# edwardyang12/Dex-NERF

Hardware: AMD Instinct MI355X
Metric: rays/sec (64+128 samples) + PSNR vs ref, 400x400 scene (higher is better)
Workload: dtype bf16; 1 GPU; C2 render: 400x400 rays/step/GPU, 64 coarse + 128 fine samples, coarse+fine FlexibleNeRFModel D8/W256/skip4 + viewdirs, PE L=10/4, 20 Dex thresholds, validation mode (det. resampling, no noise)

## Files before the change

### dex-nerf_amd/csrc/mlp_device.h

```cpp
#pragma once
#include <cstdlib>
#include <utility>

#include "mlp_layout.h"

namespace dn {

typedef float f32x16 __attribute__((ext_vector_type(16)));
typedef float f32x4 __attribute__((ext_vector_type(4)));
typedef __bf16 bf16x8 __attribute__((ext_vector_type(8)));
typedef _Float16 f16x8 __attribute__((ext_vector_type(8)));

template <int N, class F, int... I>
__device__ __forceinline__ void static_for_impl(F&& f, std::integer_sequence<int, I...>) {
  (f(std::integral_constant<int, I>{}), ...);
}
template <int N, class F>
__device__ __forceinline__ void static_for(F&& f) {
  static_for_impl<N>(static_cast<F&&>(f), std::make_integer_sequence<int, N>{});
}

constexpr int kRingPhases = 5;
constexpr int kSlotBytes = kPhasePieces * kPieceBytes;
constexpr int kRingBytes = kRingPhases * kSlotBytes;
constexpr int kInRows = 10;

template <int BF16> struct Prec;
template <> struct Prec<1> {
  using BPiece = bf16x8;
  using Elem = __bf16;
  static constexpr int EPP = 8;
  static constexpr int PPT = 2;
};
template <> struct Prec<2> {
  using BPiece = f16x8;
  using Elem = _Float16;
  static constexpr int EPP = 8;
  static constexpr int PPT = 2;
};
template <> struct Prec<0> {
  using BPiece = f32x4;
  using Elem = float;
  static constexpr int EPP = 4;
  static constexpr int PPT = 4;
};
template <int BF16, int PT> constexpr int waves_of() { return (BF16 && PT == 1) ? 8 : 4; }

struct FwdParams {
  const char* packed;
  int bias_bytes;
  int total_pieces;
  int D;
  unsigned skip_mask;
  int use_viewdirs;
  int mode;
  const float* rays;
  int ray_stride;
  const float* z;
// ... 131 lines not shown
      rd_cur = rd_nxt;
      rd_nxt = ring + slot_nxt * kSlotBytes + lane16;
    }
  }

  __device__ __forceinline__ void mid_phase() {
    if constexpr (WAVES == 8 && G::LEADER_DMA) dma_phase(pend_src + PER_WAVE * kPieceBytes, pend_dst + PER_WAVE * kPieceBytes, wave < 4 ? 1u : 0u);
    else if constexpr (WAVES == 8) dma_phase(pend_src, pend_dst, wave >= 4 ? 1u : 0u);
  }

  template <bool EVEN>
  __device__ __forceinline__ void phase_begin2() {
    if constexpr (EVEN) {
      asm volatile("s_waitcnt vmcnt(0)" ::: "memory");
      __builtin_amdgcn_s_barrier();
      advance_issue();
      dma_phase(pend_src, pend_dst, wave < 4 ? 1u : 0u);
      dma_phase(pend_src + PER_WAVE * kPieceBytes, pend_dst + PER_WAVE * kPieceBytes, wave < 4 ? 1u : 0u);
    }
    slot_nxt = (slot_nxt + 1 == kRingPhases) ? 0 : slot_nxt + 1;
    rda_cur = slot_cur_base + lane16;
    slot_cur_base = __builtin_amdgcn_readfirstlane(ring_addr + slot_nxt * kSlotBytes);
  }
  template <bool EVEN>
  __device__ __forceinline__ void mid_phase2() {
    if constexpr (EVEN) {
      advance_issue();
      dma_phase(pend_src, pend_dst, wave < 4 ? 1u : 0u);
      dma_phase(pend_src + PER_WAVE * kPieceBytes, pend_dst + PER_WAVE * kPieceBytes, wave < 4 ? 1u : 0u);
    }
  }
  unsigned long long xs_src[2];
  unsigned xs_dst[2];
  template <int PERIOD>
  __device__ __forceinline__ void xs_period_begin() {
    static_assert(PERIOD == kPhasePieces || PERIOD == 2 * kPhasePieces, "barrier period: one or two phases");
    if constexpr (PERIOD == 2 * kPhasePieces) asm volatile("s_waitcnt vmcnt(0)" ::: "memory");
    else asm volatile("s_waitcnt vmcnt(8)" ::: "memory");
    __builtin_amdgcn_s_barrier();
#pragma unroll
    for (int h = 0; h < PERIOD / kPhasePieces; ++h) {
      advance_issue();
      const unsigned long long bits = reinterpret_cast<unsigned long long>(wsrc + pend_src);
      const unsigned lo = __builtin_amdgcn_readfirstlane(static_cast<unsigned>(bits));
      const unsigned hi = __builtin_amdgcn_readfirstlane(static_cast<unsigned>(bits >> 32));
      xs_src[h] = (static_cast<unsigned long long>(hi) << 32) | lo;
      xs_dst[h] = __builtin_amdgcn_readfirstlane(ring_addr + pend_dst);
    }
  }
  template <int PERIOD, int Q>
  __device__ __forceinline__ void xs_dma_step() {
    constexpr int STEPS = PERIOD / 8;
    constexpr int H = (Q % STEPS) / 2;
    constexpr int OFF = (Q % 2) * 2048;
    unsigned keep;
    asm volatile(
        "s_cmp_lg_u32 %[wave], %[who]\n\t"
        "s_cbranch_scc1 .Ldn_xs_skip%=\n\t"
        "s_mov_b32 %[keep], m0\n\t"
        "s_mov_b32 m0, %[lds]\n\t"
        "s_nop 1\n\t"
        "global_load_lds_dwordx4 %[voff], %[sbase] offset:%[o0]\n\t"
        "global_load_lds_dwordx4 %[voff], %[sbase] offset:%[o1]\n\t"
        "s_mov_b32 m0, %[keep]\n"
        ".Ldn_xs_skip%=:"
        : [keep] "=&s"(keep)
        : [wave] "s"(wave), [who] "n"(Q / STEPS), [lds] "s"(xs_dst[H]), [voff] "v"(lane16), [sbase] "s"(xs_src[H]), [o0] "n"(OFF), [o1] "n"(OFF + 1024)
        : "memory", "scc");
  }
  template <int PERIOD, int POS>
  __device__ __forceinline__ void at_position_xs() {
    if constexpr (POS % PERIOD == 0) xs_period_begin<PERIOD>();
    if constexpr (POS % kPhasePieces == 0) {
      slot_nxt = (slot_nxt + 1 == kRingPhases) ? 0 : slot_nxt + 1;
      rda_cur = slot_cur_base + lane16;
      slot_cur_base = __builtin_amdgcn_readfirstlane(ring_addr + slot_nxt * kSlotBytes);
    }
  }
  template <int PERIOD, int POS>
  __device__ __forceinline__ void xs_after_piece() {
    if constexpr ((POS % PERIOD) < PERIOD / 2) xs_dma_step<PERIOD, POS % PERIOD>();
  }
  template <int PH, int POS>
  __device__ __forceinline__ void at_position() {
    static_assert(PH == kPhasePieces || (G::ASM_READS && G::LEADER_DMA), "the two-phase barrier period is the 48-point geometry's");
    if constexpr (POS % kPhasePieces == 0) {
      if constexpr (PH == 2 * kPhasePieces) phase_begin2<(POS % PH) == 0>();
      else phase_begin();
    }
    if constexpr (POS % kPhasePieces == kPhasePieces / 2) {
      if constexpr (PH == 2 * kPhasePieces) mid_phase2<(POS % PH) == kPhasePieces / 2>();
      else mid_phase();
    }
  }

  template <int POS, int N, int PH = kPhasePieces, bool BIAS = true>
  __device__ __forceinline__ void skip() {
    static_for<N>([&](auto i_c) {
      constexpr int pos = POS + decltype(i_c)::value;
      static_assert(pos % kPhasePieces != 0 || decltype(i_c)::value == 0, "padding never crosses a phase");
      if constexpr (pos % kPhasePieces == kPhasePieces / 2) at_position<PH, pos>();
      if constexpr (!G::ASM_READS || decltype(i_c)::value >= N - G::PREFETCH) prefetch<pos>();
    });
    settle<BIAS>();
  }

  template <int PERIOD, int POS, int N>
  __device__ __forceinline__ void skip_xs() {
    static_for<N>([&](auto i_c) {
      constexpr int pos = POS + decltype(i_c)::value;
      static_assert(pos % kPhasePieces != 0 || decltype(i_c)::value == 0, "padding never crosses a phase");
      static_assert(pos % PERIOD != 0, "padding never opens a barrier period");
      xs_after_piece<PERIOD, pos>();
      if constexpr (decltype(i_c)::value >= N - G::PREFETCH) prefetch<pos>();
    });
    settle<true>();
  }

  template <int POS>
  __device__ __forceinline__ void prefetch() {
    constexpr int q = (POS % kPhasePieces) + G::PREFETCH;
    if constexpr (G::ASM_READS) {
      const unsigned base = (q < kPhasePieces) ? rda_cur : slot_cur_base + lane16;
      asm volatile("ds_read_b128 %0, %1 offset:%2" : "=v"(af[POS % G::PREFETCH]) : "v"(base), "n"((q % kPhasePieces) * kPieceBytes));
    } else {
      const char* base = (q < kPhasePieces) ? rd_cur : rd_nxt;
      af[POS % G::PREFETCH] = *reinterpret_cast<const f32x4*>(base + (q % kPhasePieces) * kPieceBytes);
    }
  }

  template <int E>
  __device__ __forceinline__ void prologue_read() {
    asm volatile("ds_read_b128 %0, %1 offset:%2" : "=v"(af[E]) : "v"(slot_cur_base + lane16), "n"(E * kPieceBytes));
  }
  template <int POS, int NEWER>
  __device__ __forceinline__ f32x4 take() {
    asm volatile("s_waitcnt lgkmcnt(%1)" : "+v"(af[POS % G::PREFETCH]) : "n"(NEWER));
    return af[POS % G::PREFETCH];
  }
  template <int OFF>
  __device__ __forceinline__ void bias_prefetch(unsigned addr) {
    asm volatile("ds_read_b128 %0, %1 offset:%2" : "=v"(bias_nxt) : "v"(addr), "n"(OFF));
  }
  template <int NEWER>
  __device__ __forceinline__ f32x4 bias_take() {
    asm volatile("s_waitcnt lgkmcnt(%1)" : "+v"(bias_nxt) : "n"(NEWER));
// ... 266 lines not shown
```

### dex-nerf_amd/csrc/mlp_fused48_kernel.h

```cpp
#pragma once
#include "mlp_stage48.h"

namespace dn {


template <bool MAY_BE_IDENTITY = true>
__device__ __forceinline__ float pe_value(float xc, f32x4 entry) {
  const float rev = __builtin_amdgcn_fractf(xc * entry[0]) + entry[1];
  const float s = __builtin_amdgcn_sinf(rev);
  if constexpr (MAY_BE_IDENTITY) return entry[2] * xc + entry[3] * s;
  else return s;
}

__device__ __forceinline__ void rotate3(const float (&x)[3], int g, float (&xr)[3]) {
  const unsigned r = static_cast<unsigned>(g) % 3u;
  const unsigned m1 = 0u - (r & 1u), m2 = 0u - (r >> 1);
  const unsigned b0 = __float_as_uint(x[0]), b1 = __float_as_uint(x[1]), b2 = __float_as_uint(x[2]);
  xr[0] = __uint_as_float(b0 ^ ((b0 ^ b1) & m1) ^ ((b0 ^ b2) & m2));
  xr[1] = __uint_as_float(b1 ^ ((b1 ^ b2) & m1) ^ ((b1 ^ b0) & m2));
  xr[2] = __uint_as_float(b2 ^ ((b2 ^ b0) & m1) ^ ((b2 ^ b1) & m2));
}

template <int W, int F, int DC = 0, unsigned MASKC = 0, int VIEWC = 0, int SAVE = 0, int OVLP = 0, int COMP = 0>
__global__ __launch_bounds__(kG48Waves * 64, 2) void mlp_forward48_kernel(FwdParams p, G48Params q) {
// ... 76 lines not shown
    const int ln = fresh_lane();
    int pt = tile * PPG + wave * PPW + ln;
    pt = pt < n_points ? pt : n_points - 1;
    const float* r = p.rays + static_cast<long long>(pt / p.S) * p.ray_stride;
#pragma unroll
    for (int c = 0; c < 6; ++c) dma4_lanes48(r + c, inbuf_addr + c * (PPW * 4));
    dma4_lanes48(p.z + pt, inbuf_addr + 6 * (PPW * 4));
#pragma unroll
    for (int c = 0; c < 3; ++c) dma4_lanes48(r + 8 + c, inbuf_addr + (7 + c) * (PPW * 4) + set * (3 * PPW * 4));
  };

  Pipe48<WAVES> pipe;
  pipe.ring = ring;
  pipe.ring_addr = static_cast<unsigned>(reinterpret_cast<uintptr_t>((__attribute__((address_space(3))) char*)ring));
  pipe.lane16 = lane * 16;
  pipe.wsrc = q.base + q.bias_bytes + kG48TableBytes;
  pipe.total_bytes = static_cast<unsigned>(q.total_pieces) * kPieceBytes;
  pipe.q_issue = 0;
  pipe.slot_wr = 0;
  pipe.wave = wave;
#pragma unroll
  for (int ph = 0; ph < (PH == kPhasePieces ? kRingPhases - 1 : kRingPhases - 2); ++ph) pipe.issue_phase();
  if constexpr (PH == kPhasePieces) {
    g48_prologue_wait(wave);
    __builtin_amdgcn_s_barrier();
  } else {
    asm volatile("s_waitcnt vmcnt(0) lgkmcnt(0)" ::: "memory");
    __syncthreads();
  }
  pipe.slot_nxt = 0;
  auto bias_at = [&](int tile) { return pipe.ring_addr + kRingBytes + ((fresh_lane() >> 4) << 4) + tile * 64; };
  pipe.rda_cur = pipe.ring_addr + lane * 16;
  pipe.slot_cur_base = pipe.ring_addr;
  static_for<PipeGeo48::PREFETCH - 1>([&](auto e_c) { pipe.template prologue_read<decltype(e_c)::value>(); });
  pipe.template bias_prefetch<0>(bias_at(0));
  pipe.template prologue_read<PipeGeo48::PREFETCH - 1>();

  unsigned trk = 0;
  int vset = 0;
  float tfreq[OVL ? 16 : 1], tphase[OVL ? 16 : 1], tw_id[3], tw_sin[3];
  float xr_n[PT][3];
  BP8 encp;
  if constexpr (OVL) {
    const f32x4* tabx = reinterpret_cast<const f32x4*>(tab_lds) + (lane >> 4) * 16;
#pragma unroll
    for (int u = 0; u < 16; ++u) {
      const f32x4 e = tabx[u];
      tfreq[u] = e[0]; tphase[u] = e[1];
      if (u < 3) { tw_id[u] = e[2]; tw_sin[u] = e[3]; }
    }
  }
  unsigned long long idm[3] = {0ull, 0ull, 0ull};
  if constexpr (OVX) {
    const f32x4* tabx = reinterpret_cast<const f32x4*>(tab_lds) + (lane >> 4) * 16;
#pragma unroll
    for (int u = 0; u < 3; ++u) idm[u] = __ballot(tabx[u][2] != 0.0f);
  }
  const int n_tiles = static_cast<int>(p.n_tiles);
  for (int tile = blockIdx.x; tile < n_tiles; tile += gridDim.x, vset = (VSETS == 2 ? vset ^ 1 : (vset == 2 ? 0 : vset + 1))) {
    const char* act_grp[PT] = {};
    const char* mask_base = nullptr;
    if constexpr (SAVE != 0) {
      const long long wt = static_cast<long long>(tile) * WAVES + wave;
#pragma unroll
      for (int t = 0; t < PT; ++t) {
        const long long G = wt * PT + t;
        act_grp[t] = uniform_ptr(p.act + ((G >> 1) * p.act_pieces * 2 + (G & 1)) * kPieceBytes);
      }
      mask_base = uniform_ptr(p.masks + wt * p.mask_words * (2 * kPieceBytes));
    }
    const bool first_tile = tile == static_cast<int>(blockIdx.x);
    if ((!OVL && !OVX) || first_tile) {
      const int ln = fresh_lane();
      const int j = ln & 15;
      const f32x4* tabx = reinterpret_cast<const f32x4*>(tab_lds) + (ln >> 4) * 16;
      char* pex = pex_of(ln);
      if (wave >= 4) asm volatile("s_waitcnt vmcnt(0)" ::: "memory");
      float in[PT][7];
#pragma unroll
      for (int t = 0; t < PT; ++t)
#pragma unroll
        for (int c = 0; c < 7; ++c) in[t][c] = inbuf[c * PPW + t * 16 + j];
      asm volatile("s_waitcnt lgkmcnt(0)" ::: "memory");
      {
        const int nxt = tile + gridDim.x;
        if (nxt < n_tiles) issue_inputs(nxt, vset ^ 1);
      }
#pragma unroll
      for (int t = 0; t < PT; ++t) {
        float x[3];
#pragma unroll
// ... 54 lines not shown
          maskw[t][nt >> 3] = mw;
        }
      }
    };
    auto unit_tail = [&](auto nt_c, auto t_c, const auto& bo, int slot0) {
      if constexpr (SAVE != 0) {
        constexpr int nt = decltype(nt_c)::value;
        if constexpr (nt % 4 == 3) save_unit(t_c, slot0 + nt / 4, bo[nt / 2 - 1], bo[nt / 2]);
      }
    };
    auto mask_store = [&](int stage) {
      if constexpr (SAVE != 0) {
        store16_uniform_at(mask_base, static_cast<unsigned>(stage) * (2 * kPieceBytes), pipe.lane16, make_uint4(maskw[0][0], maskw[0][1], maskw[1][0], maskw[1][1]));
        if constexpr (PT == 3)
          store16_uniform_at(mask_base, static_cast<unsigned>(stage) * (2 * kPieceBytes) + kPieceBytes, pipe.lane16, make_uint4(maskw[PT - 1][0], maskw[PT - 1][1], 0u, 0u));
      }
    };
    constexpr int KHU = KH / 2;

    BP8 ba[PT][KH], bb[PT][KH];
    int bias_tile = 0;
    float out4[PT][4];
    if constexpr (XS) {
      static_assert(DC >= 2 && KDP == 1, "a trunk behind layer1; the view-direction panel is one piece");
      constexpr int PX = PH;
      f32x4 pacc[PT];
      auto nothing = [&](auto) {};
      {
        BP8 pe[PT][KXP];
#pragma unroll
        for (int t = 0; t < PT; ++t)
#pragma unroll
          for (int k = 0; k < KXP; ++k) pe[t][k] = pe_xyz(t, k);
        run_stage48x<F, PX, NT, KXP, 0, 0, false, 0, 6, 0, 0>(pipe, pe, no_pe, bias_at(0), 0u, pacc,
            [&](auto nt_c, auto s_c) { hidden_op48<F, false, decltype(nt_c)::value, decltype(s_c)::value>(pacc, ba); }, nothing);
      }
      bias_tile += NT;
      static_for<DC - 1>([&](auto i_c) {
        constexpr int i = decltype(i_c)::value;
        constexpr int P0 = xs_trunk_pos(i, NT, KH, KXP, MASKC) % PX;
        auto& bin = (i % 2 == 0) ? ba : bb;
        auto& bout = (i % 2 == 0) ? bb : ba;
        auto ops = [&](auto nt_c, auto s_c) { hidden_op48<F, true, decltype(nt_c)::value, decltype(s_c)::value>(pacc, bout); };
        auto pend = [&](auto s_c) { hidden_op48<F, (i > 0), NT - 1, decltype(s_c)::value>(pacc, bin); };
        constexpr int PN = i > 0 ? 12 : 6;
        constexpr int BY = (NT - 1) / 2;
        if constexpr ((MASKC >> i) & 1u) {
          BP8 pe[PT][KXP];
#pragma unroll
          for (int t = 0; t < PT; ++t)
#pragma unroll
            for (int k = 0; k < KXP; ++k) pe[t][k] = pe_xyz(t, k);
          run_stage48x<F, PX, NT, KH, KXP, P0, false, 0, 12, PN, BY, (i == 0 ? 2 : 1)>(pipe, bin, [&](int t, int k) { return pe[t][k]; }, bias_at(bias_tile), 0u, pacc, ops, pend, &trk);
        } else {
          run_stage48x<F, PX, NT, KH, 0, P0, false, 0, 12, PN, BY, (i == 0 ? 2 : 1)>(pipe, bin, no_pe, bias_at(bias_tile), 0u, pacc, ops, pend, &trk);
        }
        bias_tile += NT;
      });
      auto& hx = ((DC - 1) % 2 == 0) ? ba : bb;
      auto& hy = ((DC - 1) % 2 == 0) ? bb : ba;
      constexpr int POS_A = xs_trunk_pos(DC - 1, NT, KH, KXP, MASKC) % PX;
      run_stage48x<F, PX, 1, KH, 0, POS_A, false, 0, 3, (DC > 1 ? 12 : 6), (NT - 1) / 2>(pipe, hx, no_pe, bias_at(bias_tile), 0u, pacc,
          [&](auto, auto s_c) { constexpr int t = decltype(s_c)::value; pick_op48(out4[t][3], pacc[t][0]); },
          [&](auto s_c) { hidden_op48<F, (DC > 1), NT - 1, decltype(s_c)::value>(pacc, hx); });
      constexpr int POS_F = (POS_A + KH) % PX;
      run_stage48x<F, PX, NT, KH, 0, POS_F, false, 0, 12, 3, KH, 1>(pipe, hx, no_pe, bias_at(bias_tile + 1), 0u, pacc,
          [&](auto nt_c, auto s_c) { hidden_op48<F, true, decltype(nt_c)::value, decltype(s_c)::value>(pacc, hy); },
          [&](auto s_c) { constexpr int t = decltype(s_c)::value; pick_op48(out4[t][3], pacc[t][0]); }, &trk);
      bias_tile += NT + 1;
      __builtin_amdgcn_sched_barrier(0);
      {
        const int ln = fresh_lane();
        const int j = ln & 15;
        const f32x4* tabd = reinterpret_cast<const f32x4*>(tab_lds + 1024) + (ln >> 4) * 8;
        char* pex = pex_of(ln);
        static_for<PT>([&](auto t_c) {
          constexpr int t = decltype(t_c)::value;
          float v[3];
#pragma unroll
          for (int c = 0; c < 3; ++c) v[c] = inbuf[(7 + 3 * vset + c) * PPW + t * 16 + j];
          float vr[3];
          rotate3(v, ln >> 4, vr);
          BP8 piece;
#pragma unroll
          for (int e = 0; e < 8; ++e) piece[e] = static_cast<Elem>((e < 3) ? pe_value<true>(vr[e % 3], tabd[e]) : pe_value<false>(vr[e % 3], tabd[e]));
          *reinterpret_cast<BP8*>(pex + t * kPieceBytes) = piece;
          __builtin_amdgcn_sched_barrier(0);
        });
      }
      __builtin_amdgcn_sched_barrier(0);
      constexpr int POS_D = (POS_F + NT * KH) % PX;
      constexpr int KT_D = KH + KDP;
      BP8 bg[PT][KH / 2];
      BP8 ped[PT];
      typedef float f32x2 __attribute__((ext_vector_type(2)));
      float ev[2] = {0.0f, 0.0f};
      f32x2 tbl[2] = {{0.0f, 0.0f}, {0.0f, 0.0f}};
      unsigned tab_addr_v = 0u, stash_addr_v = 0u;
      float in_n[PT][7];
      if constexpr (OVX) {
        static_assert(kEncOps <= enc_begin((NT / 2) * KT_D, KT_D), "the view-direction stage has a gap for every encoding op");
        {
          const unsigned must_wait = __builtin_amdgcn_readfirstlane(wave >= 4 ? 1u : 0u);
          asm volatile("s_cmp_eq_u32 %0, 0\n\t"
                       "s_cbranch_scc1 .Ldn_ovx_nowait%=\n\t"
                       "s_waitcnt vmcnt(0)\n"
                       ".Ldn_ovx_nowait%=:" ::"s"(must_wait) : "scc", "memory");
        }
        const int ln = fresh_lane();
        const int j = ln & 15;
#pragma unroll
        for (int t = 0; t < PT; ++t)
#pragma unroll
          for (int c = 0; c < 7; ++c) in_n[t][c] = inbuf[c * PPW + t * 16 + j];
        tab_addr_v = pipe.ring_addr + kRingBytes + static_cast<unsigned>(q.bias_bytes) + static_cast<unsigned>(ln >> 4) * 256u;
        stash_addr_v = pipe.ring_addr + kRingBytes + static_cast<unsigned>(q.bias_bytes) + kG48TableBytes + wave * (PT * KXP * kPieceBytes) + static_cast<unsigned>(ln) * 16u;
        asm volatile("ds_read_b64 %0, %1" : "=v"(tbl[0]) : "v"(tab_addr_v));
      }
#pragma unroll
      for (int t = 0; t < PT; ++t) ped[t] = *reinterpret_cast<const BP8*>(pex_of(pipe.lane16 >> 4) + t * kPieceBytes);
      asm volatile("s_waitcnt lgkmcnt(0)" : "+v"(ped[0]), "+v"(ped[1]), "+v"(ped[2]), "+v"(pipe.af[0]), "+v"(pipe.af[1]), "+v"(pipe.bias_nxt), "+v"(tbl[0]));
      if constexpr (OVX) {
        const int t2 = tile + 2 * static_cast<int>(gridDim.x);
        issue_inputs_flat(t2 < n_tiles ? t2 : tile, vset);
        const int ln = fresh_lane();
#pragma unroll
        for (int t = 0; t < PT; ++t) {
          float x[3];
#pragma unroll
          for (int c = 0; c < 3; ++c) x[c] = in_n[t][c] + in_n[t][3 + c] * in_n[t][6];
          rotate3(x, ln >> 4, xr_n[t]);
        }
      }
      auto enc_hook = [&](auto b_c, auto w_c) {
        if constexpr (OVX) {
          constexpr int b = decltype(b_c)::value, w = decltype(w_c)::value;
          constexpr int q0 = enc_begin(b, KT_D), cap = enc_cap(b, KT_D);
          auto one = [&](auto q_c) {
            constexpr int qq = decltype(q_c)::value;
            if constexpr (qq < kEncOps) {
              constexpr int mt = enc_table_slot_at(qq);
// ... 3 lines not shown
              if constexpr (mt >= 0) {
                f32x2& dst = tbl[mt & 1];
                asm volatile("ds_read_b64 %0, %1 offset:%2" : "=v"(dst) : "v"(ta), "n"((mt % 16) * 16));
              }
              const float xc = xr_n[tq][u % 3];
              float& val = ev[e & 1];
              const f32x2 entry = tbl[m & 1];
              if constexpr (kind == kEncMul) asm volatile("v_mul_f32 %0, %1, %2" : "=v"(val) : "v"(xc), "v"(entry[0]));
              else if constexpr (kind == kEncFract) asm volatile("v_fract_f32 %0, %0" : "+v"(val));
              else if constexpr (kind == kEncAdd) asm volatile("v_add_f32 %0, %0, %1" : "+v"(val) : "v"(entry[1]));
              else if constexpr (kind == kEncSin) asm volatile("v_sin_f32 %0, %0" : "+v"(val));
              else if constexpr (kind == kEncSel) {
                const unsigned long long im = idm[u < 3 ? u : 0];
                asm volatile("v_cndmask_b32 %0, %0, %1, %2" : "+v"(val) : "v"(xc), "s"(im));
              } else if constexpr (kind == kEncCvt) {
                typedef unsigned u32x4 __attribute__((ext_vector_type(4)));
                const float lo = ev[0], hi = ev[1];
                unsigned dw;
                if constexpr (F == 1) asm volatile("v_cvt_pk_bf16_f32 %0, %1, %2" : "=v"(dw) : "v"(lo), "v"(hi));
                else asm volatile("v_cvt_pk_f16_f32 %0, %1, %2" : "=v"(dw) : "v"(lo), "v"(hi));
                u32x4 pw = __builtin_bit_cast(u32x4, encp);
                pw[e / 2] = dw;
                encp = __builtin_bit_cast(BP8, pw);
              } else {
                const BP8 piece = encp;
                asm volatile("ds_write_b128 %0, %1 offset:%2" : : "v"(sa), "v"(piece), "n"((tq * KXP + k2) * kPieceBytes));
              }
            }
          };
          if constexpr (w < 2) one(std::integral_constant<int, q0 + w>{});
          else if constexpr (w == 2) static_for<cap - 2>([&](auto j_c) { one(std::integral_constant<int, q0 + 2 + decltype(j_c)::value>{}); });
        }
      };
      run_stage48x<F, PX, NT / 2, KH, KDP, POS_D, false, 0, 12, 12, (NT - 1) / 2, 1>(pipe, hy, [&](int t, int) { return ped[t]; }, bias_at(bias_tile), 0u, pacc,
          [&](auto nt_c, auto s_c) { hidden_op48<F, true, decltype(nt_c)::value, decltype(s_c)::value>(pacc, bg); },
          [&](auto s_c) { hidden_op48<F, true, NT - 1, decltype(s_c)::value>(pacc, hy); }, &trk, enc_hook);
      bias_tile += NT / 2;
      constexpr int POS_R = (POS_D + (NT / 2) * (KH + KDP)) % PX;
      constexpr int END = POS_R + KH / 2;
      static_assert(END <= PX && (END - 1) / kPhasePieces == POS_R / kPhasePieces, "the tail stays inside one phase");
      constexpr int PAD_R = (kPhasePieces - END % kPhasePieces) % kPhasePieces;
      static_assert((END + PAD_R) % PX == 0, "a tile pass is a whole number of barrier periods");
      run_stage48x<F, PX, 1, KH / 2, 0, POS_R, true, PAD_R, 9, 12, (NT / 2 - 1) / 2, 1>(pipe, bg, no_pe, bias_at(bias_tile), bias_at(0), pacc,
          [&](auto, auto s_c) { constexpr int sv = decltype(s_c)::value; pick_op48(out4[sv / 3][sv % 3], pacc[sv / 3][sv % 3]); },
          [&](auto s_c) { hidden_op48<F, true, NT / 2 - 1, decltype(s_c)::value>(pacc, bg); }, &trk);
      if constexpr (PAD_R != 0) pipe.template skip_xs<PX, END, PAD_R>();
      else pipe.settle();
      asm volatile("s_nop 7\n\ts_nop 1" ::: "memory");
      static_for<9>([&](auto s_c) { constexpr int sv = decltype(s_c)::value; pick_op48(out4[sv / 3][sv % 3], pacc[sv / 3][sv % 3]); });
    } else {
    {
      BP8 pe[PT][KXP];
#pragma unroll
      for (int t = 0; t < PT; ++t)
#pragma unroll
        for (int k = 0; k < KXP; ++k) pe[t][k] = pe_xyz(t, k);
      run_stage48<F, NT, KXP, 0, 0, false, ST, 0, PH>(pipe, pe, no_pe, bias_at(0), 0u, [&](auto nt_c, auto t_c, const f32x4& acc) {
        emit48<F, false, decltype(nt_c)::value>(acc, ba[decltype(t_c)::value]);
        unit_tail(nt_c, t_c, ba[decltype(t_c)::value], p.slot_layer1);
      });
    }
    bias_tile += NT;
    if constexpr (OVL) {
      {
        const unsigned must_wait = __builtin_amdgcn_readfirstlane((wave >= 4 || first_tile) ? 1u : 0u);
        asm volatile("s_cmp_eq_u32 %0, 0\n\t"
                     "s_cbranch_scc1 .Ldn_ovl_nowait%=\n\t"
                     "s_waitcnt vmcnt(0)\n"
                     ".Ldn_ovl_nowait%=:" ::"s"(must_wait) : "scc", "memory");
      }
      const int ln = fresh_lane();
      const int j = ln & 15;
      float in[PT][7];
#pragma unroll
      for (int t = 0; t < PT; ++t)
#pragma unroll
        for (int c = 0; c < 7; ++c) in[t][c] = inbuf[c * PPW + t * 16 + j];
      asm volatile("s_waitcnt lgkmcnt(0)" ::: "memory");
      {
// ... 174 lines not shown
          f32x4 o;
          o[0] = out4[t][0]; o[1] = out4[t][1]; o[2] = out4[t][2]; o[3] = out4[t][3];
          stage[wave * PPW + t * 16 + lo] = o;
        }
      }
      asm volatile("s_waitcnt lgkmcnt(0)" ::: "memory");
      __builtin_amdgcn_s_barrier();
      const int S = p.S;
      const int rays_per_tile = PPG / S;
      for (int r = wave; r < rays_per_tile; r += WAVES) {
        const long long ray = static_cast<long long>(tile) * rays_per_tile + r;
        if (ray < q.comp.n_rays) {
          const f32x4* rows = stage + r * S;
          composite_ray([&](int sc) { const f32x4 r = rows[sc]; return make_float4(r[0], r[1], r[2], r[3]); }, p.z + ray * S,
                        p.rays + ray * p.ray_stride + 3, ray, lo, static_cast<const float*>(nullptr), 0.0f, q.comp.white, q.comp.th,
                        q.comp.n_thres, q.comp.n_rays, S, q.comp.rgb, q.comp.disp, q.comp.acc, q.comp.weights, q.comp.depth, q.comp.dex,
                        q.comp.nonfinite, RngRef{nullptr, 0u});
        }
      }
      asm volatile("s_waitcnt lgkmcnt(0)" ::: "memory");
      __builtin_amdgcn_s_barrier();
    } else {
#pragma unroll
      for (int t = 0; t < PT; ++t) {
        const int pt = tile * PPG + wave * PPW + t * 16 + (lo & 15);
        if (pt < n_points && lo < 16) {
          f32x4 o;
          o[0] = out4[t][0]; o[1] = out4[t][1]; o[2] = out4[t][2]; o[3] = out4[t][3];
          __builtin_nontemporal_store(o, reinterpret_cast<f32x4*>(p.out + static_cast<long long>(pt) * 4));
        }
      }
    }
  }
  asm volatile("s_waitcnt vmcnt(0) lgkmcnt(0)" ::: "memory");
  if constexpr (F == 2) {
    const bool out_of_range = (trk & 0xFFFFu) >= 0x7C00u || (trk >> 16) >= 0x7C00u;
    if (p.range_flag != nullptr && __ballot(out_of_range) != 0ull && (threadIdx.x & 63) == 0) atomicAdd(p.range_flag, 1u);
  }
}

#define DN_FWD48_PAPER_BF16(X)  \
  X(256, 1, 8, 0x10u, 1, 0, 2, 0) X(256, 1, 8, 0x10u, 1, 0, 0, 0)
#define DN_FWD48_PAPER_FP16(X)  \
  X(256, 2, 8, 0x10u, 1, 0, 2, 0) X(256, 2, 8, 0x10u, 1, 0, 0, 0)
#define DN_FWD48_W128(X)  \
  X(128, 1, 0, 0u, 0, 0, 0, 0) X(128, 2, 0, 0u, 0, 0, 0, 0)  \
  X(128, 1, 4, 0u, 1, 0, 0, 0) X(128, 2, 4, 0u, 1, 0, 0, 0)  \
  X(128, 1, 4, 0u, 1, 0, 1, 0) X(128, 2, 4, 0u, 1, 0, 1, 0)  \
  X(128, 1, 4, 0u, 1, 0, 0, 1) X(128, 2, 4, 0u, 1, 0, 0, 1)  \
  X(128, 1, 4, 0u, 1, 2, 0, 0) X(128, 1, 4, 0u, 1, 3, 0, 0) X(128, 1, 0, 0u, 0, 2, 0, 0)
#define DN_FWD48_W256_RT(X)  \
  X(256, 1, 0, 0u, 0, 0, 0, 0) X(256, 2, 0, 0u, 0, 0, 0, 0) X(256, 1, 0, 0u, 0, 2, 0, 0)
#define DN_FWD48_PAPER_COMP(X)  \
  X(256, 1, 8, 0x10u, 1, 0, 0, 1) X(256, 2, 8, 0x10u, 1, 0, 0, 1)
#define DN_FWD48_PAPER_TRAIN(X)  \
  X(256, 1, 8, 0x10u, 1, 2, 0, 0) X(256, 1, 8, 0x10u, 1, 3, 0, 0)
#define DN_FWD48_INSTANCES(X) \
  DN_FWD48_PAPER_BF16(X) DN_FWD48_PAPER_FP16(X) DN_FWD48_W128(X) DN_FWD48_W256_RT(X) DN_FWD48_PAPER_COMP(X) DN_FWD48_PAPER_TRAIN(X)
#define DN_FWD48_DENSITY(X) \
  X(256, 1, 8, 0x10u, 0, 0, 0, 0) X(256, 2, 8, 0x10u, 0, 0, 0, 0) X(128, 1, 4, 0u, 0, 0, 0, 0) X(128, 2, 4, 0u, 0, 0, 0, 0)

#define DN_FWD48_INSTANTIATE(W, F, DC, MASKC, VIEWC, SAVE, OVLP, COMP) \
  template __global__ void mlp_forward48_kernel<W, F, DC, MASKC, VIEWC, SAVE, OVLP, COMP>(FwdParams, G48Params);
#define DN_FWD48_EXTERN(W, F, DC, MASKC, VIEWC, SAVE, OVLP, COMP) extern DN_FWD48_INSTANTIATE(W, F, DC, MASKC, VIEWC, SAVE, OVLP, COMP)

}
```

### dex-nerf_amd/csrc/mlp_fused48_paper_bf16.hip

```cpp
#include "mlp_fused48_kernel.h"
namespace dn { DN_FWD48_PAPER_BF16(DN_FWD48_INSTANTIATE) }
```

### dex-nerf_amd/csrc/mlp_fused48_paper_fp16.hip

```cpp
#include "mlp_fused48_kernel.h"
namespace dn { DN_FWD48_PAPER_FP16(DN_FWD48_INSTANTIATE) }
```

### dex-nerf_amd/csrc/mlp_stage48.h

```cpp
#pragma once
#include <type_traits>
#include "mlp_geo48.h"

namespace dn {

using PipeGeo48 = PipeGeometry<true, true, true, 2>;
template <int WAVES>
using Pipe48 = PipeT<WAVES, PipeGeo48>;

__device__ __forceinline__ void g48_prologue_wait(unsigned wave) {
  const unsigned fetcher = __builtin_amdgcn_readfirstlane(wave < 4 ? 1u : 0u);
  asm volatile("s_cmp_eq_u32 %0, 0\n\t"
               "s_cbranch_scc1 .Ldn_prol_all%=\n\t"
               "s_waitcnt vmcnt(8) lgkmcnt(0)\n\t"
               "s_branch .Ldn_prol_done%=\n"
               ".Ldn_prol_all%=:\n\t"
               "s_waitcnt vmcnt(0) lgkmcnt(0)\n"
               ".Ldn_prol_done%=:" ::"s"(fetcher) : "scc", "memory");
}

template <int F>
__device__ __forceinline__ f32x4 mfma48(typename Prec<F>::BPiece a, typename Prec<F>::BPiece b, f32x4 c) {
  if constexpr (F == 1) return __builtin_amdgcn_mfma_f32_16x16x32_bf16(a, b, c, 0, 0, 0);
  else return __builtin_amdgcn_mfma_f32_16x16x32_f16(a, b, c, 0, 0, 0);
// ... 134 lines not shown
}
constexpr int kEncSlots = 48;
constexpr int kEncOps = enc_first(kEncSlots);
constexpr int enc_slot_of(int q) {
  int m = 0;
  while (m < kEncSlots && q >= enc_slot_len(m % 16)) { q -= enc_slot_len(m % 16); ++m; }
  return m;
}
enum { kEncMul = 0, kEncFract = 1, kEncAdd = 2, kEncSin = 3, kEncSel = 4, kEncCvt = 5, kEncWrite = 6 };
constexpr int enc_kind(int u, int idx) {
  if (idx < 4) return idx;
  int j = 4;
  if (u < 3) { if (idx == j) return kEncSel; ++j; }
  if ((u % 8) % 2) { if (idx == j) return kEncCvt; ++j; }
  return kEncWrite;
}
constexpr int enc_cap(int b, int kt) { return (b % kt) >= 6 ? 4 : 3; }
constexpr int enc_begin(int b, int kt) {
  int q = 0;
  for (int i = 0; i < b; ++i) q += enc_cap(i, kt);
  return q;
}
constexpr int kEncLead = 5;
constexpr int enc_table_slot_at(int q) {
  for (int m = 1; m < kEncSlots; ++m)
    if (enc_first(m) - kEncLead == q) return m;
  return -1;
}

struct XsNoHook {
  template <class B, class W>
  __device__ __forceinline__ void operator()(B, W) const {}
};
template <int F, int PX, int NT_OUT, int KH, int KP, int POS0, bool LAST, int PAD, int NOPS, int PEND_N, int PEND_BY, int TRK = 0, class PipeT, class BH,
          class BP, class Ops, class Pend, class Hook = XsNoHook>
__device__ __forceinline__ void run_stage48x(PipeT& pipe, const BH& bh, BP&& bp, unsigned bias_addr, unsigned next_addr, f32x4 (&pacc)[3],
                                             Ops&& ops, Pend&& pend, unsigned* trk = nullptr, Hook&& hook = Hook{}) {
  constexpr int PT = 3, KT = KH + KP;
  static_assert(KT >= 2 && KH >= 1, "the bias prefetch distance assumes at least two pieces per tile; a tile's first piece is a hidden piece");
  static_for<NT_OUT>([&](auto nt_c) {
    constexpr int nt = decltype(nt_c)::value;
    constexpr int NP = nt == 0 ? PEND_N : NOPS;
    constexpr int E = xs_blocks(NP, KT, nt == 0 ? PEND_BY : KT);
    constexpr int PER = xs_per(NP, E);
    static_assert(PER * E >= NP, "every pending op has a slot");
    constexpr int TOT = (F == 2 && TRK != 0) ? PT * KH * 4 : 0;
    constexpr int Q0 = nt * TOT / NT_OUT, Q1 = (nt + 1) * TOT / NT_OUT;
    constexpr int NTRK = (TRK == 2) ? (Q1 - Q0) : (Q1 - Q0 + 1) / 2;
    constexpr int TB = KT - E > 0 ? KT - E : 1;
    constexpr int TPER = (NTRK + TB - 1) / TB;
    auto run_op = [&](auto s_c) {
      constexpr int sidx = decltype(s_c)::value;
      if constexpr (sidx < NP) {
        if constexpr (nt == 0) pend(s_c);
        else ops(std::integral_constant<int, nt - 1>{}, s_c);
      }
    };
    auto run_trk = [&](auto q_c) {
      constexpr int qi = decltype(q_c)::value;
      if constexpr (qi < NTRK) {
        typedef unsigned u32x4 __attribute__((ext_vector_type(4)));
        auto dword = [&](int q) { return __builtin_bit_cast(u32x4, bh[q / (KH * 4)][(q / 4) % KH])[q % 4]; };
        unsigned tv = *trk;
        if constexpr (TRK == 2) {
          const unsigned v = dword(Q0 + qi);
          unsigned tmp;
          asm volatile("v_and_b32 %1, 0x7fff7fff, %2\n\tv_pk_max_u16 %0, %0, %1" : "+v"(tv), "=&v"(tmp) : "v"(v));
        } else {
          constexpr int qa = Q0 + 2 * qi, qb = (qa + 1 < Q1) ? qa + 1 : qa;
          const unsigned va = dword(qa), vb = dword(qb);
          asm volatile("v_pk_maximum3_f16 %0, %0, %1, %2" : "+v"(tv) : "v"(va), "v"(vb));
        }
        *trk = tv;
      }
    };
    f32x4 acc[PT];
    static_for<KT>([&](auto k_c) {
      constexpr int k = decltype(k_c)::value;
      constexpr int pos = POS0 + nt * KT + k;
      pipe.template at_position_xs<PX, pos>();
      f32x4 b = {0.0f, 0.0f, 0.0f, 0.0f};
      if constexpr (k == 0) b = pipe.template bias_take<1>();
      constexpr int newer = g48_issued<LAST, POS0 + NT_OUT * KT, PAD>(pos + 1, pos + PipeGeo48::PREFETCH) + ((k == KT - 1) ? 1 : 0);
      f32x4& a = pipe.af[pos % PipeGeo48::PREFETCH];
      static_for<PT>([&](auto t_c) {
        constexpr int t = decltype(t_c)::value;
        if constexpr (t == 0) {
          if constexpr (k == 0) mfma48_first_w<F, newer>(acc[t], a, bh[t][0], b);
          else if constexpr (k < KH) mfma48_acc_w<F, newer>(acc[t], a, bh[t][k]);
          else mfma48_acc_w<F, newer>(acc[t], a, bp(t, k - KH));
        } else if constexpr (k == 0) mfma48_first<F>(acc[t], a, bh[t][0], b);
        else if constexpr (k < KH) mfma48_acc<F>(acc[t], a, bh[t][k]);
        else mfma48_acc<F>(acc[t], a, bp(t, k - KH));
        if constexpr (k < E) {
          if constexpr (t < 2) run_op(std::integral_constant<int, k * PER + t>{});
          else static_for<(PER > 2 ? PER - 2 : 0)>([&](auto j_c) { run_op(std::integral_constant<int, k * PER + 2 + decltype(j_c)::value>{}); });
        } else if constexpr (NTRK > 0) {
          constexpr int kb = (KT - E > 0) ? k - E : 0;
          if constexpr (t < 2) run_trk(std::integral_constant<int, kb * TPER + t>{});
          else static_for<(TPER > 2 ? TPER - 2 : 0)>([&](auto j_c) { run_trk(std::integral_constant<int, kb * TPER + 2 + decltype(j_c)::value>{}); });
        }
        hook(std::integral_constant<int, nt * KT + k>{}, t_c);
      });
      if constexpr (KT - E <= 0 && NTRK > 0 && k == KT - 1)
        static_for<NTRK>([&](auto q_c) { run_trk(q_c); });
      pipe.template xs_after_piece<PX, pos>();
      hook(std::integral_constant<int, nt * KT + k>{}, std::integral_constant<int, 3>{});
      if constexpr (g48_issued<LAST, POS0 + NT_OUT * KT, PAD>(pos + PipeGeo48::PREFETCH, pos + PipeGeo48::PREFETCH + 1) == 1) pipe.template prefetch<pos>();
      if constexpr (k == KT - 2) {
        if constexpr (nt + 1 < NT_OUT) pipe.template bias_prefetch<(nt + 1) * 64>(bias_addr);
        else if constexpr (LAST) pipe.template bias_prefetch<0>(next_addr);
        else pipe.template bias_prefetch<NT_OUT * 64>(bias_addr);
      }
    });
#pragma unroll
    for (int t = 0; t < PT; ++t) pacc[t] = acc[t];
  });
}

template <int F, bool RELU, int NT, class BO>
__device__ __forceinline__ void emit48(const f32x4& acc, BO& bo) {
  typedef float f32x2 __attribute__((ext_vector_type(2)));
  typedef typename Prec<F>::Elem e16x2 __attribute__((ext_vector_type(2)));
  typedef short s16x2 __attribute__((ext_vector_type(2)));
  typedef unsigned u32x4 __attribute__((ext_vector_type(4)));
  u32x4 w = __builtin_bit_cast(u32x4, bo[NT / 2]);
#pragma unroll
  for (int d = 0; d < 2; ++d) {
    f32x2 f = {acc[2 * d], acc[2 * d + 1]};
    e16x2 v = __builtin_convertvector(f, e16x2);
    if constexpr (RELU) {
      s16x2 bits = __builtin_bit_cast(s16x2, v);
      const s16x2 zero = {0, 0};
      bits = __builtin_elementwise_max(bits, zero);
      v = __builtin_bit_cast(e16x2, bits);
    }
    w[(NT & 1) * 2 + d] = __builtin_bit_cast(unsigned, v);
  }
  bo[NT / 2] = __builtin_bit_cast(typename Prec<F>::BPiece, w);
// ... 5 lines not shown
```

Before: 5.378 million rays/s.

## Compile separate fetcher and consumer tile loops for W256 cross-stage weight streaming

The whole tile loop is now templated on a wave role. Waves 0-3 compile a fetcher path that issues the global-to-LDS weight DMA and computes its addresses. Waves 4+ compile a consumer path with the DMA steps and address setup removed at compile time, and the in-stage encoding wait becomes unconditional for consumers instead of a runtime scalar branch. This removes per-piece scalar compares and branches and lowers register pressure on consumer waves, at the cost of duplicated code, larger binaries, and the paper instantiations split into separate compilation units.

```diff
diff --git a/dex-nerf_amd/csrc/mlp_device.h b/dex-nerf_amd/csrc/mlp_device.h
--- a/dex-nerf_amd/csrc/mlp_device.h
+++ b/dex-nerf_amd/csrc/mlp_device.h
@@ -24,6 +24,7 @@
 constexpr int kSlotBytes = kPhasePieces * kPieceBytes;
 constexpr int kRingBytes = kRingPhases * kSlotBytes;
 constexpr int kInRows = 10;
+enum { kXsFetcher = 0, kXsConsumer = 1 };
 
 template <int BF16> struct Prec;
 template <> struct Prec<1> {
@@ -221,20 +222,22 @@
   }
   unsigned long long xs_src[2];
   unsigned xs_dst[2];
-  template <int PERIOD>
+  template <int PERIOD, int ROLE = kXsFetcher>
   __device__ __forceinline__ void xs_period_begin() {
     static_assert(PERIOD == kPhasePieces || PERIOD == 2 * kPhasePieces, "barrier period: one or two phases");
     if constexpr (PERIOD == 2 * kPhasePieces) asm volatile("s_waitcnt vmcnt(0)" ::: "memory");
     else asm volatile("s_waitcnt vmcnt(8)" ::: "memory");
     __builtin_amdgcn_s_barrier();
-#pragma unroll
-    for (int h = 0; h < PERIOD / kPhasePieces; ++h) {
-      advance_issue();
-      const unsigned long long bits = reinterpret_cast<unsigned long long>(wsrc + pend_src);
-      const unsigned lo = __builtin_amdgcn_readfirstlane(static_cast<unsigned>(bits));
-      const unsigned hi = __builtin_amdgcn_readfirstlane(static_cast<unsigned>(bits >> 32));
-      xs_src[h] = (static_cast<unsigned long long>(hi) << 32) | lo;
-      xs_dst[h] = __builtin_amdgcn_readfirstlane(ring_addr + pend_dst);
+    if constexpr (ROLE == kXsFetcher) {
+#pragma unroll
+      for (int h = 0; h < PERIOD / kPhasePieces; ++h) {
+        advance_issue();
+        const unsigned long long bits = reinterpret_cast<unsigned long long>(wsrc + pend_src);
+        const unsigned lo = __builtin_amdgcn_readfirstlane(static_cast<unsigned>(bits));
+        const unsigned hi = __builtin_amdgcn_readfirstlane(static_cast<unsigned>(bits >> 32));
+        xs_src[h] = (static_cast<unsigned long long>(hi) << 32) | lo;
+        xs_dst[h] = __builtin_amdgcn_readfirstlane(ring_addr + pend_dst);
+      }
     }
   }
   template <int PERIOD, int Q>
@@ -257,18 +260,18 @@
         : [wave] "s"(wave), [who] "n"(Q / STEPS), [lds] "s"(xs_dst[H]), [voff] "v"(lane16), [sbase] "s"(xs_src[H]), [o0] "n"(OFF), [o1] "n"(OFF + 1024)
         : "memory", "scc");
   }
-  template <int PERIOD, int POS>
+  template <int PERIOD, int POS, int ROLE = kXsFetcher>
   __device__ __forceinline__ void at_position_xs() {
-    if constexpr (POS % PERIOD == 0) xs_period_begin<PERIOD>();
+    if constexpr (POS % PERIOD == 0) xs_period_begin<PERIOD, ROLE>();
     if constexpr (POS % kPhasePieces == 0) {
       slot_nxt = (slot_nxt + 1 == kRingPhases) ? 0 : slot_nxt + 1;
       rda_cur = slot_cur_base + lane16;
       slot_cur_base = __builtin_amdgcn_readfirstlane(ring_addr + slot_nxt * kSlotBytes);
     }
   }
-  template <int PERIOD, int POS>
+  template <int PERIOD, int POS, int ROLE = kXsFetcher>
   __device__ __forceinline__ void xs_after_piece() {
-    if constexpr ((POS % PERIOD) < PERIOD / 2) xs_dma_step<PERIOD, POS % PERIOD>();
+    if constexpr (ROLE == kXsFetcher && (POS % PERIOD) < PERIOD / 2) xs_dma_step<PERIOD, POS % PERIOD>();
   }
   template <int PH, int POS>
   __device__ __forceinline__ void at_position() {
@@ -294,13 +297,13 @@
     settle<BIAS>();
   }
 
-  template <int PERIOD, int POS, int N>
+  template <int PERIOD, int POS, int N, int ROLE = kXsFetcher>
   __device__ __forceinline__ void skip_xs() {
     static_for<N>([&](auto i_c) {
       constexpr int pos = POS + decltype(i_c)::value;
       static_assert(pos % kPhasePieces != 0 || decltype(i_c)::value == 0, "padding never crosses a phase");
       static_assert(pos % PERIOD != 0, "padding never opens a barrier period");
-      xs_after_piece<PERIOD, pos>();
+      xs_after_piece<PERIOD, pos, ROLE>();
       if constexpr (decltype(i_c)::value >= N - G::PREFETCH) prefetch<pos>();
     });
     settle<true>();
diff --git a/dex-nerf_amd/csrc/mlp_fused48_kernel.h b/dex-nerf_amd/csrc/mlp_fused48_kernel.h
--- a/dex-nerf_amd/csrc/mlp_fused48_kernel.h
+++ b/dex-nerf_amd/csrc/mlp_fused48_kernel.h
@@ -132,9 +132,13 @@
   auto bias_at = [&](int tile) { return pipe.ring_addr + kRingBytes + ((fresh_lane() >> 4) << 4) + tile * 64; };
   pipe.rda_cur = pipe.ring_addr + lane * 16;
   pipe.slot_cur_base = pipe.ring_addr;
-  static_for<PipeGeo48::PREFETCH - 1>([&](auto e_c) { pipe.template prologue_read<decltype(e_c)::value>(); });
-  pipe.template bias_prefetch<0>(bias_at(0));
-  pipe.template prologue_read<PipeGeo48::PREFETCH - 1>();
+  constexpr bool SPLIT = XS && W == 256;
+  auto first_reads = [&]() {
+    static_for<PipeGeo48::PREFETCH - 1>([&](auto e_c) { pipe.template prologue_read<decltype(e_c)::value>(); });
+    pipe.template bias_prefetch<0>(bias_at(0));
+    pipe.template prologue_read<PipeGeo48::PREFETCH - 1>();
+  };
+  if constexpr (!SPLIT) first_reads();
 
   unsigned trk = 0;
   int vset = 0;
@@ -157,6 +161,9 @@
     for (int u = 0; u < 3; ++u) idm[u] = __ballot(tabx[u][2] != 0.0f);
   }
   const int n_tiles = static_cast<int>(p.n_tiles);
+  auto tile_loop = [&](auto role_c) __attribute__((always_inline)) {
+  constexpr int ROLE = decltype(role_c)::value;
+  if constexpr (SPLIT) first_reads();
   for (int tile = blockIdx.x; tile < n_tiles; tile += gridDim.x, vset = (VSETS == 2 ? vset ^ 1 : (vset == 2 ? 0 : vset + 1))) {
     const char* act_grp[PT] = {};
     const char* mask_base = nullptr;
@@ -277,7 +284,7 @@
         for (int t = 0; t < PT; ++t)
 #pragma unroll
           for (int k = 0; k < KXP; ++k) pe[t][k] = pe_xyz(t, k);
-        run_stage48x<F, PX, NT, KXP, 0, 0, false, 0, 6, 0, 0>(pipe, pe, no_pe, bias_at(0), 0u, pacc,
+        run_stage48x<ROLE, F, PX, NT, KXP, 0, 0, false, 0, 6, 0, 0>(pipe, pe, no_pe, bias_at(0), 0u, pacc,
             [&](auto nt_c, auto s_c) { hidden_op48<F, false, decltype(nt_c)::value, decltype(s_c)::value>(pacc, ba); }, nothing);
       }
       bias_tile += NT;
@@ -296,20 +303,20 @@
           for (int t = 0; t < PT; ++t)
 #pragma unroll
             for (int k = 0; k < KXP; ++k) pe[t][k] = pe_xyz(t, k);
-          run_stage48x<F, PX, NT, KH, KXP, P0, false, 0, 12, PN, BY, (i == 0 ? 2 : 1)>(pipe, bin, [&](int t, int k) { return pe[t][k]; }, bias_at(bias_tile), 0u, pacc, ops, pend, &trk);
+          run_stage48x<ROLE, F, PX, NT, KH, KXP, P0, false, 0, 12, PN, BY, (i == 0 ? 2 : 1)>(pipe, bin, [&](int t, int k) { return pe[t][k]; }, bias_at(bias_tile), 0u, pacc, ops, pend, &trk);
         } else {
-          run_stage48x<F, PX, NT, KH, 0, P0, false, 0, 12, PN, BY, (i == 0 ? 2 : 1)>(pipe, bin, no_pe, bias_at(bias_tile), 0u, pacc, ops, pend, &trk);
+          run_stage48x<ROLE, F, PX, NT, KH, 0, P0, false, 0, 12, PN, BY, (i == 0 ? 2 : 1)>(pipe, bin, no_pe, bias_at(bias_tile), 0u, pacc, ops, pend, &trk);
         }
         bias_tile += NT;
       });
       auto& hx = ((DC - 1) % 2 == 0) ? ba : bb;
       auto& hy = ((DC - 1) % 2 == 0) ? bb : ba;
       constexpr int POS_A = xs_trunk_pos(DC - 1, NT, KH, KXP, MASKC) % PX;
-      run_stage48x<F, PX, 1, KH, 0, POS_A, false, 0, 3, (DC > 1 ? 12 : 6), (NT - 1) / 2>(pipe, hx, no_pe, bias_at(bias_tile), 0u, pacc,
+      run_stage48x<ROLE, F, PX, 1, KH, 0, POS_A, false, 0, 3, (DC > 1 ? 12 : 6), (NT - 1) / 2>(pipe, hx, no_pe, bias_at(bias_tile), 0u, pacc,
           [&](auto, auto s_c) { constexpr int t = decltype(s_c)::value; pick_op48(out4[t][3], pacc[t][0]); },
           [&](auto s_c) { hidden_op48<F, (DC > 1), NT - 1, decltype(s_c)::value>(pacc, hx); });
       constexpr int POS_F = (POS_A + KH) % PX;
-      run_stage48x<F, PX, NT, KH, 0, POS_F, false, 0, 12, 3, KH, 1>(pipe, hx, no_pe, bias_at(bias_tile + 1), 0u, pacc,
+      run_stage48x<ROLE, F, PX, NT, KH, 0, POS_F, false, 0, 12, 3, KH, 1>(pipe, hx, no_pe, bias_at(bias_tile + 1), 0u, pacc,
           [&](auto nt_c, auto s_c) { hidden_op48<F, true, decltype(nt_c)::value, decltype(s_c)::value>(pacc, hy); },
           [&](auto s_c) { constexpr int t = decltype(s_c)::value; pick_op48(out4[t][3], pacc[t][0]); }, &trk);
       bias_tile += NT + 1;
@@ -345,13 +352,9 @@
       float in_n[PT][7];
       if constexpr (OVX) {
         static_assert(kEncOps <= enc_begin((NT / 2) * KT_D, KT_D), "the view-direction stage has a gap for every encoding op");
-        {
-          const unsigned must_wait = __builtin_amdgcn_readfirstlane(wave >= 4 ? 1u : 0u);
-          asm volatile("s_cmp_eq_u32 %0, 0\n\t"
-                       "s_cbranch_scc1 .Ldn_ovx_nowait%=\n\t"
-                       "s_waitcnt vmcnt(0)\n"
-                       ".Ldn_ovx_nowait%=:" ::"s"(must_wait) : "scc", "memory");
-        }
+        static_assert(SPLIT, "in-stage encoding: an instance whose pass is compiled per role");
+        if constexpr (ROLE == kXsConsumer) asm volatile("s_waitcnt vmcnt(0)" ::: "memory");
+        else asm volatile("" ::: "memory");
         const int ln = fresh_lane();
         const int j = ln & 15;
 #pragma unroll
@@ -421,7 +424,7 @@
           else if constexpr (w == 2) static_for<cap - 2>([&](auto j_c) { one(std::integral_constant<int, q0 + 2 + decltype(j_c)::value>{}); });
         }
       };
-      run_stage48x<F, PX, NT / 2, KH, KDP, POS_D, false, 0, 12, 12, (NT - 1) / 2, 1>(pipe, hy, [&](int t, int) { return ped[t]; }, bias_at(bias_tile), 0u, pacc,
+      run_stage48x<ROLE, F, PX, NT / 2, KH, KDP, POS_D, false, 0, 12, 12, (NT - 1) / 2, 1>(pipe, hy, [&](int t, int) { return ped[t]; }, bias_at(bias_tile), 0u, pacc,
           [&](auto nt_c, auto s_c) { hidden_op48<F, true, decltype(nt_c)::value, decltype(s_c)::value>(pacc, bg); },
           [&](auto s_c) { hidden_op48<F, true, NT - 1, decltype(s_c)::value>(pacc, hy); }, &trk, enc_hook);
       bias_tile += NT / 2;
@@ -430,10 +433,10 @@
       static_assert(END <= PX && (END - 1) / kPhasePieces == POS_R / kPhasePieces, "the tail stays inside one phase");
       constexpr int PAD_R = (kPhasePieces - END % kPhasePieces) % kPhasePieces;
       static_assert((END + PAD_R) % PX == 0, "a tile pass is a whole number of barrier periods");
-      run_stage48x<F, PX, 1, KH / 2, 0, POS_R, true, PAD_R, 9, 12, (NT / 2 - 1) / 2, 1>(pipe, bg, no_pe, bias_at(bias_tile), bias_at(0), pacc,
+      run_stage48x<ROLE, F, PX, 1, KH / 2, 0, POS_R, true, PAD_R, 9, 12, (NT / 2 - 1) / 2, 1>(pipe, bg, no_pe, bias_at(bias_tile), bias_at(0), pacc,
           [&](auto, auto s_c) { constexpr int sv = decltype(s_c)::value; pick_op48(out4[sv / 3][sv % 3], pacc[sv / 3][sv % 3]); },
           [&](auto s_c) { hidden_op48<F, true, NT / 2 - 1, decltype(s_c)::value>(pacc, bg); }, &trk);
-      if constexpr (PAD_R != 0) pipe.template skip_xs<PX, END, PAD_R>();
+      if constexpr (PAD_R != 0) pipe.template skip_xs<PX, END, PAD_R, ROLE>();
       else pipe.settle();
       asm volatile("s_nop 7\n\ts_nop 1" ::: "memory");
       static_for<9>([&](auto s_c) { constexpr int sv = decltype(s_c)::value; pick_op48(out4[sv / 3][sv % 3], pacc[sv / 3][sv % 3]); });
@@ -674,6 +677,13 @@
       }
     }
   }
+  };
+  if constexpr (SPLIT) {
+    if (wave < 4) tile_loop(std::integral_constant<int, kXsFetcher>{});
+    else tile_loop(std::integral_constant<int, kXsConsumer>{});
+  } else {
+    tile_loop(std::integral_constant<int, kXsFetcher>{});
+  }
   asm volatile("s_waitcnt vmcnt(0) lgkmcnt(0)" ::: "memory");
   if constexpr (F == 2) {
     const bool out_of_range = (trk & 0xFFFFu) >= 0x7C00u || (trk >> 16) >= 0x7C00u;
@@ -681,10 +691,12 @@
   }
 }
 
-#define DN_FWD48_PAPER_BF16(X)  \
-  X(256, 1, 8, 0x10u, 1, 0, 2, 0) X(256, 1, 8, 0x10u, 1, 0, 0, 0)
-#define DN_FWD48_PAPER_FP16(X)  \
-  X(256, 2, 8, 0x10u, 1, 0, 2, 0) X(256, 2, 8, 0x10u, 1, 0, 0, 0)
+#define DN_FWD48_PAPER_BF16_ENC(X) X(256, 1, 8, 0x10u, 1, 0, 2, 0)
+#define DN_FWD48_PAPER_BF16_PLAIN(X) X(256, 1, 8, 0x10u, 1, 0, 0, 0)
+#define DN_FWD48_PAPER_FP16_ENC(X) X(256, 2, 8, 0x10u, 1, 0, 2, 0)
+#define DN_FWD48_PAPER_FP16_PLAIN(X) X(256, 2, 8, 0x10u, 1, 0, 0, 0)
+#define DN_FWD48_PAPER_BF16(X) DN_FWD48_PAPER_BF16_ENC(X) DN_FWD48_PAPER_BF16_PLAIN(X)
+#define DN_FWD48_PAPER_FP16(X) DN_FWD48_PAPER_FP16_ENC(X) DN_FWD48_PAPER_FP16_PLAIN(X)
 #define DN_FWD48_W128(X)  \
   X(128, 1, 0, 0u, 0, 0, 0, 0) X(128, 2, 0, 0u, 0, 0, 0, 0)  \
   X(128, 1, 4, 0u, 1, 0, 0, 0) X(128, 2, 4, 0u, 1, 0, 0, 0)  \
diff --git a/dex-nerf_amd/csrc/mlp_fused48_paper_bf16.hip b/dex-nerf_amd/csrc/mlp_fused48_paper_bf16.hip
--- a/dex-nerf_amd/csrc/mlp_fused48_paper_bf16.hip
+++ b/dex-nerf_amd/csrc/mlp_fused48_paper_bf16.hip
@@ -1,2 +1,2 @@
 #include "mlp_fused48_kernel.h"
-namespace dn { DN_FWD48_PAPER_BF16(DN_FWD48_INSTANTIATE) }
+namespace dn { DN_FWD48_PAPER_BF16_ENC(DN_FWD48_INSTANTIATE) }
diff --git a/dex-nerf_amd/csrc/mlp_fused48_paper_bf16_plain.hip b/dex-nerf_amd/csrc/mlp_fused48_paper_bf16_plain.hip
--- /dev/null
+++ b/dex-nerf_amd/csrc/mlp_fused48_paper_bf16_plain.hip
@@ -0,0 +1,2 @@
+#include "mlp_fused48_kernel.h"
+namespace dn { DN_FWD48_PAPER_BF16_PLAIN(DN_FWD48_INSTANTIATE) }
diff --git a/dex-nerf_amd/csrc/mlp_fused48_paper_fp16.hip b/dex-nerf_amd/csrc/mlp_fused48_paper_fp16.hip
--- a/dex-nerf_amd/csrc/mlp_fused48_paper_fp16.hip
+++ b/dex-nerf_amd/csrc/mlp_fused48_paper_fp16.hip
@@ -1,2 +1,2 @@
 #include "mlp_fused48_kernel.h"
-namespace dn { DN_FWD48_PAPER_FP16(DN_FWD48_INSTANTIATE) }
+namespace dn { DN_FWD48_PAPER_FP16_ENC(DN_FWD48_INSTANTIATE) }
diff --git a/dex-nerf_amd/csrc/mlp_fused48_paper_fp16_plain.hip b/dex-nerf_amd/csrc/mlp_fused48_paper_fp16_plain.hip
--- /dev/null
+++ b/dex-nerf_amd/csrc/mlp_fused48_paper_fp16_plain.hip
@@ -0,0 +1,2 @@
+#include "mlp_fused48_kernel.h"
+namespace dn { DN_FWD48_PAPER_FP16_PLAIN(DN_FWD48_INSTANTIATE) }
diff --git a/dex-nerf_amd/csrc/mlp_stage48.h b/dex-nerf_amd/csrc/mlp_stage48.h
--- a/dex-nerf_amd/csrc/mlp_stage48.h
+++ b/dex-nerf_amd/csrc/mlp_stage48.h
@@ -190,8 +190,8 @@
   template <class B, class W>
   __device__ __forceinline__ void operator()(B, W) const {}
 };
-template <int F, int PX, int NT_OUT, int KH, int KP, int POS0, bool LAST, int PAD, int NOPS, int PEND_N, int PEND_BY, int TRK = 0, class PipeT, class BH,
-          class BP, class Ops, class Pend, class Hook = XsNoHook>
+template <int ROLE, int F, int PX, int NT_OUT, int KH, int KP, int POS0, bool LAST, int PAD, int NOPS, int PEND_N, int PEND_BY, int TRK = 0, class PipeT,
+          class BH, class BP, class Ops, class Pend, class Hook = XsNoHook>
 __device__ __forceinline__ void run_stage48x(PipeT& pipe, const BH& bh, BP&& bp, unsigned bias_addr, unsigned next_addr, f32x4 (&pacc)[3],
                                              Ops&& ops, Pend&& pend, unsigned* trk = nullptr, Hook&& hook = Hook{}) {
   constexpr int PT = 3, KT = KH + KP;
@@ -236,7 +236,7 @@
     static_for<KT>([&](auto k_c) {
       constexpr int k = decltype(k_c)::value;
       constexpr int pos = POS0 + nt * KT + k;
-      pipe.template at_position_xs<PX, pos>();
+      pipe.template at_position_xs<PX, pos, ROLE>();
       f32x4 b = {0.0f, 0.0f, 0.0f, 0.0f};
       if constexpr (k == 0) b = pipe.template bias_take<1>();
       constexpr int newer = g48_issued<LAST, POS0 + NT_OUT * KT, PAD>(pos + 1, pos + PipeGeo48::PREFETCH) + ((k == KT - 1) ? 1 : 0);
@@ -262,7 +262,7 @@
       });
       if constexpr (KT - E <= 0 && NTRK > 0 && k == KT - 1)
         static_for<NTRK>([&](auto q_c) { run_trk(q_c); });
-      pipe.template xs_after_piece<PX, pos>();
+      pipe.template xs_after_piece<PX, pos, ROLE>();
       hook(std::integral_constant<int, nt * KT + k>{}, std::integral_constant<int, 3>{});
       if constexpr (g48_issued<LAST, POS0 + NT_OUT * KT, PAD>(pos + PipeGeo48::PREFETCH, pos + PipeGeo48::PREFETCH + 1) == 1) pipe.template prefetch<pos>();
       if constexpr (k == KT - 2) {
```

Result: faster. 5.463 million rays/s, median of 6 (+1.6%).
